# chayanchatterjee/GW-Whisper

Measured on AMD Instinct MI355X. Metric: 1s-strain segments/sec (encoder fwd), higher is better.
Workload: dtype bf16; 1 GPU; whisper-tiny encoder fwd, batch 256 log-mel (80x3000) per GPU, 1500 tokens, random-init weights (BASELINE configs[1]); global_batch=256, parallelism=dp1, encoder=tiny, streams_per_gpu=1

## Files before the change

__graft_entry__.py:

```python

from __future__ import annotations

import os
import subprocess
import sys

ROOT = os.path.dirname(os.path.abspath(__file__))
if ROOT not in sys.path:
    sys.path.insert(0, ROOT)


def build() -> None:
    csrc = os.path.join(ROOT, "gw_whisper_amd", "csrc")
    subprocess.run(["make", "-C", csrc, "-j", str(min(8, os.cpu_count() or 1))], check=True)
    asm = os.path.join(csrc, "build", "mlp_fused.s")
    subprocess.run(["/opt/rocm/bin/hipcc", "-O3", "-std=c++17", "--offload-arch=gfx950", "-ffp-contract=fast", "-mllvm",
                    "-pragma-unroll-threshold=4000000", "-S", "--cuda-device-only", os.path.join(csrc, "mlp_fused.hip"),
                    "-o", asm], check=True)
    subprocess.run([sys.executable, os.path.join(ROOT, "tools", "audit_asm_loads.py"), asm, "k_mlp_fused"], check=True)
    subprocess.run([sys.executable, os.path.join(ROOT, "tools", "audit_asm_mfma.py"), asm, "k_mlp_fused"], check=True)
    subprocess.run([sys.executable, os.path.join(ROOT, "tools", "audit_spills.py"), asm, "k_mlp_fused", "ILi1ELb1=4", "ILi3ELb1=10",
                    "ILi0ELb1=2", "ILi1ELb0=29"], check=True)
    asm4 = os.path.join(csrc, "build", "gemm_v4.s")
    subprocess.run(["/opt/rocm/bin/hipcc", "-O3", "-std=c++17", "--offload-arch=gfx950", "-ffp-contract=fast", "-S",
                    "--cuda-device-only", os.path.join(csrc, "gemm_v4.hip"), "-o", asm4], check=True)
    subprocess.run([sys.executable, os.path.join(ROOT, "tools", "audit_asm_preload.py"), asm4, "k_gemm_bf16_v4ILi2E"], check=True)
    for k in ("k_gemm_bf16_v4ILi0E", "k_gemm_bf16_v4ILi1E"):
        subprocess.run([sys.executable, os.path.join(ROOT, "tools", "audit_asm_preload.py"), asm4, k, "--no-loads"], check=True)
    for k in ("k_gemm_bf16_v4ILi3E", "k_gemm_bf16_v4ILi16E"):
        subprocess.run([sys.executable, os.path.join(ROOT, "tools", "audit_asm_preload.py"), asm4, k, "--scratch-only"], check=True)
    asmc = os.path.join(csrc, "build", "classify.s")
    subprocess.run(["/opt/rocm/bin/hipcc", "-O3", "-std=c++17", "--offload-arch=gfx950", "-ffp-contract=fast", "-S",
                    "--cuda-device-only", os.path.join(csrc, "classify.hip"), "-o", asmc], check=True)
    for k in ("k_head_fwd", "k_head_bwd_in", "k_head_bwd_w", "k_eval_accumulate"):
        subprocess.run([sys.executable, os.path.join(ROOT, "tools", "audit_asm_preload.py"), asmc, k, "--scratch-only"], check=True)
    asmd = os.path.join(csrc, "build", "detect.s")
    subprocess.run(["/opt/rocm/bin/hipcc", "-O3", "-std=c++17", "--offload-arch=gfx950", "-ffp-contract=fast", "-S",
                    "--cuda-device-only", os.path.join(csrc, "detect.hip"), "-o", asmd], check=True)
    for k in ("k_det_fwdILin1E", "k_det_fwdILi0E", "k_det_fwdILi1E", "k_det_bwd_in", "k_det_bwd_w", "k_det_eval",
              "k_sel_hist", "k_sel_pick", "k_det_counts"):
        subprocess.run([sys.executable, os.path.join(ROOT, "tools", "audit_asm_preload.py"), asmd, k, "--scratch-only"], check=True)
    asmr = os.path.join(csrc, "build", "roc.s")
    subprocess.run(["/opt/rocm/bin/hipcc", "-O3", "-std=c++17", "--offload-arch=gfx950", "-ffp-contract=off", "-S",
                    "--cuda-device-only", os.path.join(csrc, "roc.hip"), "-o", asmr], check=True)
    for k in ("k_roc_keys", "k_roc_hist", "k_roc_scan", "k_roc_scatter", "k_roc_finish", "k_roc_groups", "k_roc_curve",
              "k_roc_bootstrap", "k_roc_band", "k_bin_eval"):
        subprocess.run([sys.executable, os.path.join(ROOT, "tools", "audit_asm_preload.py"), asmr, k, "--scratch-only"], check=True)
    import gw_whisper_amd
    lib = gw_whisper_amd.lib()
    assert lib.gww_version() >= 107


def smoke() -> None:
    import numpy as np
    import torch

    from gw_whisper_amd import ops, synth
    from gw_whisper_amd.encoder import WhisperConfig, WhisperEncoder
    from oracle import encoder as oenc
    from oracle import logmel as olm

    assert torch.cuda.is_available(), "smoke() needs a GPU"
    dev = torch.device("cuda:0")
    wave = synth.strain_segments(2, seed=21)
    mel = ops.logmel(torch.from_numpy(wave).to(dev))
    mel_ref = olm.log_mel(wave)
    err_mel = float(np.abs(mel.cpu().numpy() - mel_ref).max())
    assert err_mel < 1e-4, f"log-mel mismatch {err_mel}"

    cfg = WhisperConfig(128, 2, 2, 512)
    sd = synth.encoder_state_dict(128, 2, 2, 512, seed=3)
    ref = oenc.encoder_forward(sd, mel_ref, oenc.EncCfg(128, 2, 2, 512))
    for prec, tol in (("fp32", 2e-3), ("bf16", 6e-2)):
        enc = WhisperEncoder.from_numpy_state_dict(sd, cfg, precision=prec).to(dev)
        with torch.no_grad():
            out = enc(mel).last_hidden_state
            last = enc.last_token(mel)
        torch.cuda.synchronize()
        err = float(np.abs(out.cpu().numpy() - ref).max())
        err_last = float(np.abs(last.cpu().numpy() - ref[:, -1]).max())
        print(f"smoke[{prec}]: max|hidden - oracle| = {err:.3e}, last-token {err_last:.3e}, log-mel {err_mel:.3e}")
        assert err < tol and err_last < tol, f"encoder[{prec}] mismatch {err} / {err_last}"
    d, L, H, F = synth.ENCODER_SIZES["tiny"]
    sd = synth.encoder_state_dict(d, L, H, F, seed=5)
    ref = oenc.encoder_forward(sd, mel_ref[:1], oenc.EncCfg(d, L, H, F), dtype=np.float32)
    enc = WhisperEncoder.from_numpy_state_dict(sd, WhisperConfig.named("tiny"), precision="bf16").to(dev)
    with torch.no_grad():
        out = enc(mel[:1]).last_hidden_state
    torch.cuda.synchronize()
    err = float(np.abs(out.cpu().numpy() - ref).max())
    print(f"smoke[tiny bf16]: max|hidden - oracle| = {err:.3e} (|hidden| max {np.abs(ref).max():.2f})")
    assert err < 0.15, f"whisper-tiny bf16 mismatch {err}"
    print("smoke OK")


if __name__ == "__main__":
    {"build": build, "smoke": smoke}[sys.argv[1] if len(sys.argv) > 1 else "build"]()
```

gw_whisper_amd/csrc/attention.hip:

```cpp
#include "common.h"

#include <stdlib.h>
#include <type_traits>

#ifndef GWW_ATT_EPI16
#define GWW_ATT_EPI16 1
#endif
namespace gww {

#ifdef GWW_STAMP
__device__ unsigned long long g_stamp_att[8];
#define ASTAMP_DECL unsigned long long _t0 = __builtin_amdgcn_s_memtime(); unsigned long long _acc[7] = {0, 0, 0, 0, 0, 0, 0};
#define ASTAMP(i)                                                  \
  do {                                                             \
    __builtin_amdgcn_sched_barrier(0);                             \
    const unsigned long long _t1 = __builtin_amdgcn_s_memtime();   \
    _acc[i] += _t1 - _t0;                                          \
    _t0 = _t1;                                                     \
    __builtin_amdgcn_sched_barrier(0);                             \
  } while (0)
#define ASTAMP_FLUSH                                                                 \
  if (lane == 0) {                                                                   \
    for (int _q = 0; _q < 7; ++_q) atomicAdd(&g_stamp_att[_q], _acc[_q]);            \
    atomicAdd(&g_stamp_att[7], 1ull);                                                \
// ... 355 lines not shown
    }
#pragma unroll
    for (int g = 0; g < 2; ++g)
#pragma unroll
      for (int j = 0; j < 16; ++j) st[g][j] = __builtin_amdgcn_exp2f(st[g][j]);
    if constexpr (LATE) { if (kt + 1 < n_kt) gload(kt + 1); }
    if constexpr (VSUM) {
      float ps = 0.f;
#pragma unroll
      for (int g = 0; g < 2; ++g)
#pragma unroll
        for (int j = 0; j < 16; ++j) ps += st[g][j];
      l_run += ps;
    }
#pragma unroll
    for (int g = 0; g < 2; ++g) {
#pragma unroll
      for (int s = 0; s < 2; ++s) {
        const bf16x8 pf = cvt8(st[g], 8 * s);
        if constexpr (!VSUM) lt = __builtin_amdgcn_mfma_f32_32x32x16_bf16(ones, pf, lt, 0, 0, 0);
#pragma unroll
        for (int n = 0; n < 2; ++n) {
          const unsigned char* vb = vbase[n] + BUF * TILE_BYTES + (32 * g + 16 * s) * 128;
          const bf16x4 lo4 = __builtin_amdgcn_ds_read_tr16_b64_v4bf16((lds_bf16x4_ptr)vb);
          const bf16x4 hi4 = __builtin_amdgcn_ds_read_tr16_b64_v4bf16((lds_bf16x4_ptr)(vb + 8 * 128));
          bf16x8 vf;
          vf[0] = lo4[0]; vf[1] = lo4[1]; vf[2] = lo4[2]; vf[3] = lo4[3];
          vf[4] = hi4[0]; vf[5] = hi4[1]; vf[6] = hi4[2]; vf[7] = hi4[3];
          ot[n] = __builtin_amdgcn_mfma_f32_32x32x16_bf16(vf, pf, ot[n], 0, 0, 0);
        }
      }
    }
    if (kt + 1 < n_kt) lstore(std::integral_constant<int, BUF ^ 1>{});
    __syncthreads();
  };
  using P0 = std::integral_constant<int, 0>;
  using P1 = std::integral_constant<int, 1>;
  using Yes = std::true_type;
  using No = std::false_type;

  gload(0);
  lstore(P0{});
  __syncthreads();
  const bool ragged = (T % KB) != 0;
  if (n_kt == 1) {
    if (ragged) tile(0, P0{}, Yes{}, Yes{});
    else tile(0, P0{}, Yes{}, No{});
  } else {
    tile(0, P0{}, Yes{}, No{});
    int kt = 1;
    for (; kt + 2 <= n_kt - 1; kt += 2) {
      tile(kt, P1{}, No{}, No{});
      tile(kt + 1, P0{}, No{}, No{});
    }
    if (kt == n_kt - 2) {
      tile(kt, P1{}, No{}, No{});
      if (ragged) tile(kt + 1, P0{}, No{}, Yes{});
      else tile(kt + 1, P0{}, No{}, No{});
    } else {
      if (ragged) tile(kt, P1{}, No{}, Yes{});
      else tile(kt, P1{}, No{}, No{});
    }
  }

  const float l_tot = (VAR & 2) ? l_run + __shfl_xor(l_run, 32, 64) : lt[0];
  const float inv = 1.0f / l_tot;
  if (lse && q_row < T && hh == 0)
    lse[((long)b * H + h) * T + q_row] = (m_run + __log2f(l_tot)) * 0.69314718055994530942f;
  if (q_row < T) {
    unsigned short* orow = ctx + ((long)b * T + q_row) * d + h * DH;
#pragma unroll
    for (int n = 0; n < 2; ++n)
#pragma unroll
      for (int c = 0; c < 4; ++c) {
        const int dh = 32 * n + 8 * c + 4 * hh;
        u32x2 o = {pack2bf(ot[n][4 * c] * inv, ot[n][4 * c + 1] * inv),
                   pack2bf(ot[n][4 * c + 2] * inv, ot[n][4 * c + 3] * inv)};
        *reinterpret_cast<u32x2*>(orow + dh) = o;
      }
  }
}

#endif
#ifndef GWW_ATT_NBUF
#define GWW_ATT_NBUF 2
#endif
template <int MINW, bool MSUM, bool NOMAX>
__global__ __launch_bounds__(256, MINW) void k_attention_dma_bf16(const unsigned short* __restrict__ qkv,
                                                                 unsigned short* __restrict__ ctx,
                                                                 float* __restrict__ lse, int T, int H, int q_tiles,
                                                                 int qt0) {
  constexpr int NB = GWW_ATT_NBUF;
  __shared__ __attribute__((aligned(16))) unsigned char lds[NB * 2 * KB * DH * 2];
  constexpr int TILE_BYTES = KB * DH * 2, NW = 4;
  typedef __attribute__((address_space(3))) void* lds_ptr;
  typedef const __attribute__((address_space(1))) void* g_ptr;
  const int tid = threadIdx.x, lane = tid & 63, wave = tid >> 6;
  const int wave_u = __builtin_amdgcn_readfirstlane(wave);
  const unsigned nblk = gridDim.x, per = nblk >> 3;
  const unsigned wid = blockIdx.x < 8 * per ? (blockIdx.x & 7) * per + (blockIdx.x >> 3) : blockIdx.x;
  const int qt = qt0 + wid % q_tiles;
  const int bh = wid / q_tiles;
  const int b = bh / H, h = bh - b * H;
  const int d = H * DH;
  const long row_stride = 3L * d;
  const unsigned short* base = qkv + (long)b * T * row_stride;
  const unsigned short* qp = base + h * DH;
  const unsigned short* kp = base + d + h * DH;
  const unsigned short* vp = base + 2 * d + h * DH;
  const int r = lane & 31, hh = lane >> 5;
  const int q_row = qt * (NW * 32) + wave * 32 + r;
  const int q_ld = q_row < T ? q_row : T - 1;
  const bool wave_live = qt * (NW * 32) + wave_u * 32 < T;
  bf16x8 qf[4];
#pragma unroll
  for (int s = 0; s < 4; ++s) qf[s] = *reinterpret_cast<const bf16x8*>(qp + (long)q_ld * row_stride + 16 * s + 8 * hh);

  const int n_kt = (T + KB - 1) / KB;
  const bool ragged = (T % KB) != 0;
  unsigned koff[2], voff[2];
#pragma unroll
  for (int j = 0; j < 2; ++j) {
    const int row = 8 * (2 * wave + j) + (lane >> 3), pos = lane & 7;
    koff[j] = (unsigned)(row * (int)row_stride * 2 + ((pos ^ ((row >> 1) & 7)) << 4));
    voff[j] = (unsigned)(row * (int)row_stride * 2 + ((pos ^ (((row >> 1) & 1) << 2)) << 4));
  }
  auto dma = [&](int kt, auto buf_c) {
    constexpr int BUF = decltype(buf_c)::value;
    const char* kb = reinterpret_cast<const char*>(kp + (long)kt * KB * row_stride);
    const char* vb = reinterpret_cast<const char*>(vp + (long)kt * KB * row_stride);
    unsigned char* dk = lds + BUF * TILE_BYTES + (2 * wave_u) * 1024;
    unsigned char* dv = dk + NB * TILE_BYTES;
    if constexpr (NB == 3) {
      const unsigned mk = (unsigned)(unsigned long long)(lds_ptr)dk, mv = (unsigned)(unsigned long long)(lds_ptr)dv;
      unsigned ko[2], vo[2];
      if (kt != n_kt - 1 || !ragged) {
        ko[0] = koff[0]; ko[1] = koff[1]; vo[0] = voff[0]; vo[1] = voff[1];
      } else {
        const int last_row = T - 1 - kt * KB;
#pragma unroll
        for (int j = 0; j < 2; ++j) {
          const int row = 8 * (2 * wave + j) + (lane >> 3), pos = lane & 7;
          const int rc = row < last_row ? row : last_row;
          ko[j] = (unsigned)(rc * (int)row_stride * 2 + ((pos ^ ((row >> 1) & 7)) << 4));
          vo[j] = (unsigned)(rc * (int)row_stride * 2 + ((pos ^ (((row >> 1) & 1) << 2)) << 4));
        }
      }
#pragma unroll
      for (int j = 0; j < 2; ++j) {
        asm volatile("s_mov_b32 m0, %2\n\ts_nop 0\n\tglobal_load_lds_dwordx4 %0, %1" : : "v"(ko[j]), "s"(kb), "s"(mk + 1024u * j) : "memory");
        asm volatile("s_mov_b32 m0, %2\n\ts_nop 0\n\tglobal_load_lds_dwordx4 %0, %1" : : "v"(vo[j]), "s"(vb), "s"(mv + 1024u * j) : "memory");
      }
    } else if (kt != n_kt - 1 || !ragged) {
#pragma unroll
      for (int j = 0; j < 2; ++j) {
        __builtin_amdgcn_global_load_lds((g_ptr)(kb + koff[j]), (lds_ptr)(dk + j * 1024), 16, 0, 0);
        __builtin_amdgcn_global_load_lds((g_ptr)(vb + voff[j]), (lds_ptr)(dv + j * 1024), 16, 0, 0);
      }
    } else {
      const int last_row = T - 1 - kt * KB;
#pragma unroll
      for (int j = 0; j < 2; ++j) {
        const int row = 8 * (2 * wave + j) + (lane >> 3), pos = lane & 7;
        const int rc = row < last_row ? row : last_row;
        const unsigned ko = (unsigned)(rc * (int)row_stride * 2 + ((pos ^ ((row >> 1) & 7)) << 4));
        const unsigned vo = (unsigned)(rc * (int)row_stride * 2 + ((pos ^ (((row >> 1) & 1) << 2)) << 4));
// ... 114 lines not shown
      }
    }
    if constexpr (!MSUM) l_run += ps;
#pragma unroll
    for (int g = 0; g < 2; ++g) {
      if (MASKED && g == 1 && !g1_live) continue;
#pragma unroll
      for (int s = 0; s < 2; ++s) {
        const bf16x8 pf = cvt8(st[g], 8 * s);
        if constexpr (MSUM) lt = __builtin_amdgcn_mfma_f32_32x32x16_bf16(ones, pf, lt, 0, 0, 0);
#pragma unroll
        for (int n = 0; n < 2; ++n) {
          const unsigned char* vb = vbase[n] + BUF * TILE_BYTES + (32 * g + 16 * s) * 128;
          const bf16x4 lo4 = __builtin_amdgcn_ds_read_tr16_b64_v4bf16((lds_bf16x4_ptr)vb);
          const bf16x4 hi4 = __builtin_amdgcn_ds_read_tr16_b64_v4bf16((lds_bf16x4_ptr)(vb + 8 * 128));
          bf16x8 vf;
          vf[0] = lo4[0]; vf[1] = lo4[1]; vf[2] = lo4[2]; vf[3] = lo4[3];
          vf[4] = hi4[0]; vf[5] = hi4[1]; vf[6] = hi4[2]; vf[7] = hi4[3];
          ot[n] = __builtin_amdgcn_mfma_f32_32x32x16_bf16(vf, pf, ot[n], 0, 0, 0);
        }
      }
    }
    }
    if constexpr (NB == 3) {
      if (kt + 2 < n_kt) asm volatile("s_waitcnt vmcnt(4)\n\ts_barrier" ::: "memory");
      else asm volatile("s_waitcnt vmcnt(0)\n\ts_barrier" ::: "memory");
    } else {
      __syncthreads();
    }
  };
  using P0 = std::integral_constant<int, 0>;
  using P1 = std::integral_constant<int, 1>;
  using Yes = std::true_type;
  using No = std::false_type;

  if constexpr (NB == 3) {
    using P2 = std::integral_constant<int, 2>;
    dma(0, P0{});
    if (n_kt > 1) {
      dma(1, P1{});
      asm volatile("s_waitcnt vmcnt(4)\n\ts_barrier" ::: "memory");
    } else {
      asm volatile("s_waitcnt vmcnt(0)\n\ts_barrier" ::: "memory");
    }
#pragma unroll
    for (int s4 = 0; s4 < 4; ++s4) asm volatile("" : "+v"(qf[s4]));
    tile(0, P0{}, Yes{}, No{}, n_kt == 1 && ragged);
    for (int kt = 1; kt < n_kt; kt += 3) {
      tile(kt, P1{}, No{}, No{}, ragged && kt == n_kt - 1);
      if (kt + 1 < n_kt) tile(kt + 1, P2{}, No{}, No{}, ragged && kt + 1 == n_kt - 1);
      if (kt + 2 < n_kt) tile(kt + 2, P0{}, No{}, No{}, ragged && kt + 2 == n_kt - 1);
    }
  } else {
    dma(0, P0{});
    __syncthreads();
    if (n_kt == 1) {
      if (ragged) tile(0, P0{}, Yes{}, Yes{});
      else tile(0, P0{}, Yes{}, No{});
    } else {
      tile(0, P0{}, Yes{}, No{});
      int kt = 1;
      for (; kt + 2 <= n_kt - 1; kt += 2) {
        tile(kt, P1{}, No{}, No{});
        tile(kt + 1, P0{}, No{}, No{});
      }
      if (kt == n_kt - 2) {
        tile(kt, P1{}, No{}, No{});
        if (ragged) tile(kt + 1, P0{}, No{}, Yes{});
        else tile(kt + 1, P0{}, No{}, No{});
      } else {
        if (ragged) tile(kt, P1{}, No{}, Yes{});
        else tile(kt, P1{}, No{}, No{});
      }
    }
  }

  float l_tot;
  if constexpr (MSUM) {
    l_tot = lt[0];
  } else {
    const auto sw = __builtin_amdgcn_permlane32_swap(__float_as_uint(l_run), __float_as_uint(l_run), false, false);
    l_tot = __uint_as_float(sw[0]) + __uint_as_float(sw[1]);
  }
  const float inv = 1.0f / l_tot;
  if (lse && q_row < T && hh == 0)
    lse[((long)b * H + h) * T + q_row] = (m_run + __log2f(l_tot)) * 0.69314718055994530942f;
#if GWW_ATT_EPI16
  {
    unsigned short* orow = ctx + ((long)b * T + q_row) * d + h * DH;
#pragma unroll
    for (int n = 0; n < 2; ++n)
#pragma unroll
      for (int cp = 0; cp < 2; ++cp) {
        const int c0 = 2 * cp, c1 = 2 * cp + 1;
        const unsigned a0 = pack2bf(ot[n][4 * c0] * inv, ot[n][4 * c0 + 1] * inv), a1 = pack2bf(ot[n][4 * c0 + 2] * inv, ot[n][4 * c0 + 3] * inv);
        const unsigned b0 = pack2bf(ot[n][4 * c1] * inv, ot[n][4 * c1 + 1] * inv), b1 = pack2bf(ot[n][4 * c1 + 2] * inv, ot[n][4 * c1 + 3] * inv);
        const auto s0 = __builtin_amdgcn_permlane32_swap(a0, b0, false, false);
        const auto s1 = __builtin_amdgcn_permlane32_swap(a1, b1, false, false);
        u32x4 o = {s0[0], s1[0], s0[1], s1[1]};
        if (q_row < T) *reinterpret_cast<u32x4*>(orow + 32 * n + 8 * (hh ? c1 : c0)) = o;
      }
  }
#else
  if (q_row < T) {
    unsigned short* orow = ctx + ((long)b * T + q_row) * d + h * DH;
#pragma unroll
    for (int n = 0; n < 2; ++n)
#pragma unroll
      for (int c = 0; c < 4; ++c) {
        const int dh = 32 * n + 8 * c + 4 * hh;
        u32x2 o = {pack2bf(ot[n][4 * c] * inv, ot[n][4 * c + 1] * inv),
                   pack2bf(ot[n][4 * c + 2] * inv, ot[n][4 * c + 3] * inv)};
        *reinterpret_cast<u32x2*>(orow + dh) = o;
      }
  }
#endif
}

#ifdef GWW_LAB
constexpr int PP_SLOTS = 4;
#ifndef GWW_PP_PRIO
#define GWW_PP_PRIO 0
#endif
template <int MODE>
__global__ __launch_bounds__(MODE == 1 ? 256 : 512, 1) void k_attention_pp_bf16(const unsigned short* __restrict__ qkv,
                                                              unsigned short* __restrict__ ctx,
                                                              float* __restrict__ lse, int T, int H, int q_tiles,
                                                              int qt0) {
  constexpr int TILE_BYTES = KB * DH * 2;
  __shared__ __attribute__((aligned(16))) unsigned char lds[2 * PP_SLOTS * TILE_BYTES];
  typedef __attribute__((address_space(3))) void* lds_ptr;
  typedef const __attribute__((address_space(1))) void* g_ptr;
  const int tid = threadIdx.x, lane = tid & 63;
  const int wave = __builtin_amdgcn_readfirstlane(tid >> 6);
  const bool g1 = wave >= 4;
  constexpr int NWV = MODE == 1 ? 4 : 8, PPW = 8 / NWV;
  const unsigned nblk = gridDim.x, per = nblk >> 3;
  const unsigned wid = blockIdx.x < 8 * per ? (blockIdx.x & 7) * per + (blockIdx.x >> 3) : blockIdx.x;
  const int qt = qt0 + wid % q_tiles;
  const int bh = wid / q_tiles;
  const int b = bh / H, h = bh - b * H;
  const int d = H * DH;
  const long row_stride = 3L * d;
  const unsigned short* base = qkv + (long)b * T * row_stride;
  const unsigned short* qp = base + h * DH;
  const unsigned short* kp = base + d + h * DH;
  const unsigned short* vp = base + 2 * d + h * DH;
  const int r = lane & 31, hh = lane >> 5;
  const int q_row = qt * (NWV * 32) + wave * 32 + r;
  const int q_ld = q_row < T ? q_row : T - 1;
  bf16x8 qf[4];
#pragma unroll
  for (int s = 0; s < 4; ++s) qf[s] = *reinterpret_cast<const bf16x8*>(qp + (long)q_ld * row_stride + 16 * s + 8 * hh);

  const int n_kt = (T + KB - 1) / KB;
  const bool ragged = (T % KB) != 0;
  const int dpos = lane & 7;
  int drow[PPW];
  unsigned koff[PPW], voff[PPW];
#pragma unroll
  for (int j = 0; j < PPW; ++j) {
    drow[j] = 8 * (wave + NWV * j) + (lane >> 3);
    koff[j] = (unsigned)(drow[j] * (int)row_stride * 2 + ((dpos ^ ((drow[j] >> 1) & 7)) << 4));
    voff[j] = (unsigned)(drow[j] * (int)row_stride * 2 + ((dpos ^ (((drow[j] >> 1) & 1) << 2)) << 4));
  }
  auto dma = [&](int kt) {
    const char* kb = reinterpret_cast<const char*>(kp + (long)kt * KB * row_stride);
    const char* vb = reinterpret_cast<const char*>(vp + (long)kt * KB * row_stride);
    if (kt != n_kt - 1 || !ragged) {
#pragma unroll
      for (int j = 0; j < PPW; ++j) {
        unsigned char* dk = lds + (kt & (PP_SLOTS - 1)) * TILE_BYTES + (wave + NWV * j) * 1024;
        __builtin_amdgcn_global_load_lds((g_ptr)(kb + koff[j]), (lds_ptr)dk, 16, 0, 0);
        __builtin_amdgcn_global_load_lds((g_ptr)(vb + voff[j]), (lds_ptr)(dk + PP_SLOTS * TILE_BYTES), 16, 0, 0);
      }
    } else {
      const int last_row = T - 1 - kt * KB;
#pragma unroll
      for (int j = 0; j < PPW; ++j) {
        unsigned char* dk = lds + (kt & (PP_SLOTS - 1)) * TILE_BYTES + (wave + NWV * j) * 1024;
        const int rc = drow[j] < last_row ? drow[j] : last_row;
        const unsigned ko = (unsigned)(rc * (int)row_stride * 2 + ((dpos ^ ((drow[j] >> 1) & 7)) << 4));
        const unsigned vo = (unsigned)(rc * (int)row_stride * 2 + ((dpos ^ (((drow[j] >> 1) & 1) << 2)) << 4));
        __builtin_amdgcn_global_load_lds((g_ptr)(kb + ko), (lds_ptr)dk, 16, 0, 0);
        __builtin_amdgcn_global_load_lds((g_ptr)(vb + vo), (lds_ptr)(dk + PP_SLOTS * TILE_BYTES), 16, 0, 0);
      }
    }
  };

  const int tr_q = (lane & 15) >> 2, tr_p = lane & 3;
  const int tr_colbyte = (((lane & 31) >> 4) * 16 + 4 * tr_p) * 2;
  const unsigned char* kbase[4];
#pragma unroll
  for (int s = 0; s < 4; ++s) kbase[s] = lds + k_off(r, 2 * s + hh);
  const unsigned char* vbase[2];
#pragma unroll
  for (int n = 0; n < 2; ++n) vbase[n] = lds + PP_SLOTS * TILE_BYTES + v_off(4 * hh + tr_q, 64 * n + tr_colbyte);

  f32x16 ot[2], st[2];
// ... 420 lines not shown
  using No = std::false_type;
  auto tile_rt = [&](int kt, bool masked) {
    switch (kt & 3) {
      case 0: if (masked) tile(kt, std::integral_constant<int, 0>{}, No{}, Yes{}); else tile(kt, std::integral_constant<int, 0>{}, No{}, No{}); break;
      case 1: if (masked) tile(kt, std::integral_constant<int, 1>{}, No{}, Yes{}); else tile(kt, std::integral_constant<int, 1>{}, No{}, No{}); break;
      case 2: if (masked) tile(kt, std::integral_constant<int, 2>{}, No{}, Yes{}); else tile(kt, std::integral_constant<int, 2>{}, No{}, No{}); break;
      default: if (masked) tile(kt, std::integral_constant<int, 3>{}, No{}, Yes{}); else tile(kt, std::integral_constant<int, 3>{}, No{}, No{}); break;
    }
  };

  dma(0);
  if (n_kt > 1) {
    dma(1);
    asm volatile("s_waitcnt vmcnt(2)" ::: "memory");
  } else {
    asm volatile("s_waitcnt vmcnt(0)" ::: "memory");
  }
  __builtin_amdgcn_s_barrier();
  if (g1) __builtin_amdgcn_s_barrier();
  if (GWW_PP_PRIO == 2 && g1) __builtin_amdgcn_s_setprio(1);
  if (n_kt == 1 && ragged) tile(0, std::integral_constant<int, 0>{}, Yes{}, Yes{});
  else tile(0, std::integral_constant<int, 0>{}, Yes{}, No{});
  {
    int kt = 1;
    for (; kt + 4 <= n_kt - 1; kt += 4) {
      tile(kt, std::integral_constant<int, 1>{}, No{}, No{});
      tile(kt + 1, std::integral_constant<int, 2>{}, No{}, No{});
      tile(kt + 2, std::integral_constant<int, 3>{}, No{}, No{});
      tile(kt + 3, std::integral_constant<int, 0>{}, No{}, No{});
    }
    for (; kt < n_kt; ++kt) tile_rt(kt, ragged && kt == n_kt - 1);
  }
  pv_reads((n_kt - 1) & 3);
  pv_mfma();
  if (!g1) __builtin_amdgcn_s_barrier();
  ASTAMP(6);
  ASTAMP_FLUSH
  }

  float l_tot;
  {
    const auto sw = __builtin_amdgcn_permlane32_swap(__float_as_uint(l_run), __float_as_uint(l_run), false, false);
    l_tot = __uint_as_float(sw[0]) + __uint_as_float(sw[1]);
  }
  const float inv = 1.0f / l_tot;
  if (lse && q_row < T && hh == 0)
    lse[((long)b * H + h) * T + q_row] = (m_run + __log2f(l_tot)) * 0.69314718055994530942f;
  {
    unsigned short* orow = ctx + ((long)b * T + q_row) * d + h * DH;
#pragma unroll
    for (int n = 0; n < 2; ++n)
#pragma unroll
      for (int cp = 0; cp < 2; ++cp) {
        const int c0 = 2 * cp, c1 = 2 * cp + 1;
        const unsigned a0 = pack2bf(ot[n][4 * c0] * inv, ot[n][4 * c0 + 1] * inv), a1 = pack2bf(ot[n][4 * c0 + 2] * inv, ot[n][4 * c0 + 3] * inv);
        const unsigned b0 = pack2bf(ot[n][4 * c1] * inv, ot[n][4 * c1 + 1] * inv), b1 = pack2bf(ot[n][4 * c1 + 2] * inv, ot[n][4 * c1 + 3] * inv);
        const auto s0 = __builtin_amdgcn_permlane32_swap(a0, b0, false, false);
        const auto s1 = __builtin_amdgcn_permlane32_swap(a1, b1, false, false);
        u32x4 o = {s0[0], s1[0], s0[1], s1[1]};
        if (q_row < T) *reinterpret_cast<u32x4*>(orow + 32 * n + 8 * (hh ? c1 : c0)) = o;
      }
  }
}

#endif
bool attention_log2q_enabled() {
  static const bool off = lab_int("GWW_ATT_LOG2Q", 1) == 0;
  return !off;
}

int launch_attention_bf16(const void* qkv, void* ctx, int B, int T, int H, hipStream_t s, float* lse,
                          bool last_tile_only, bool q_log2) {
  GWW_REQUIRE(qkv && ctx, "attention_bf16: NULL operand");
  GWW_REQUIRE(B >= 0 && T > 0 && H > 0, "attention_bf16: bad shape B=%d T=%d H=%d", B, T, H);
  GWW_REQUIRE((((uintptr_t)qkv) & 15) == 0 && (((uintptr_t)ctx) & 15) == 0, "attention_bf16: 16-byte alignment");
  if (B == 0) return GWW_OK;
#ifdef GWW_LAB
  if (q_log2 && !last_tile_only && lab_int("GWW_ATT_W64", 0) != 0) return launch_attention_w64_bf16(qkv, ctx, B, T, H, s, lse);
#endif
  const unsigned short* in = (const unsigned short*)qkv;
  unsigned short* out = (unsigned short*)ctx;
#ifdef GWW_LAB
  const int nw_env = (int)lab_int("GWW_ATT_WAVES", 0);
  const int var_env = (int)lab_int("GWW_ATT_VAR", 7);
  const bool pp = q_log2 && var_env >= 8;
  const int nw = ((nw_env == 8 && !q_log2) || (pp && var_env == 8)) ? 8 : 4;
#else
  const int nw = 4;
#endif
  const int all_tiles = (T + nw * 32 - 1) / (nw * 32);
  const int q_tiles = last_tile_only ? 1 : all_tiles, qt0 = last_tile_only ? all_tiles - 1 : 0;
  const long blocks = (long)q_tiles * B * H;
  GWW_REQUIRE(blocks < 2147483647L, "attention_bf16: grid too large");
#define GWW_DMA(MW, MS, NM) hipLaunchKernelGGL((k_attention_dma_bf16<MW, MS, NM>), dim3((unsigned)blocks), dim3(256), 0, s, in, out, lse, T, H, q_tiles, qt0)
#ifdef GWW_LAB
  if (pp && var_env >= 9) {
    hipLaunchKernelGGL((k_attention_pp_bf16<1>), dim3((unsigned)blocks), dim3(256), 0, s, in, out, lse, T, H, q_tiles, qt0);
  } else if (pp) {
    hipLaunchKernelGGL((k_attention_pp_bf16<0>), dim3((unsigned)blocks), dim3(512), 0, s, in, out, lse, T, H, q_tiles, qt0);
  } else if (q_log2) {
    const int var = var_env & 7;
#define GWW_L2(VV) hipLaunchKernelGGL((k_attention_l2_bf16<4, VV>), dim3((unsigned)blocks), dim3(256), 0, s, in, out, lse, T, H, q_tiles, qt0)
    switch (var) {
      case 0: GWW_L2(0); break;
      case 1: GWW_L2(1); break;
      case 2: GWW_L2(2); break;
      case 3: GWW_L2(3); break;
      case 4: GWW_DMA(3, false, false); break;
      case 5: GWW_DMA(4, false, false); break;
      case 6: GWW_DMA(3, true, false); break;
      default: GWW_DMA(3, false, true); break;
    }
#undef GWW_L2
  } else if (nw == 8) {
    hipLaunchKernelGGL(k_attention_bf16<8>, dim3((unsigned)blocks), dim3(512), 0, s, in, out, lse, T, H, q_tiles, qt0);
  } else
#else
  if (q_log2) {
    GWW_DMA(3, false, true);
  } else
#endif
  {
    hipLaunchKernelGGL(k_attention_bf16<4>, dim3((unsigned)blocks), dim3(256), 0, s, in, out, lse, T, H, q_tiles, qt0);
  }
#undef GWW_DMA
  GWW_LAUNCH_CHECK();
  return GWW_OK;
}

constexpr int FKB = 32;
constexpr int FLDS = DH + 1;

__global__ __launch_bounds__(256) void k_attention_f32(const float* __restrict__ qkv, float* __restrict__ ctx,
                                                       int T, int H, int q_tiles) {
  __shared__ float Ks[FKB][FLDS];
  __shared__ float Vs[FKB][FLDS];
  const int tid = threadIdx.x, lane = tid & 63, wave = tid >> 6;
  const int qt = blockIdx.x % q_tiles;
  const int bh = blockIdx.x / q_tiles;
  const int b = bh / H, h = bh - b * H;
  const int d = H * DH;
  const long row_stride = 3L * d;
  const float* base = qkv + (long)b * T * row_stride;
  const float* qp = base + h * DH;
  const float* kp = base + d + h * DH;
  const float* vp = base + 2 * d + h * DH;
  const int r = lane & 31, hh = lane >> 5;
  const int q_row = qt * QB + wave * 32 + r;
  const int q_ld = q_row < T ? q_row : T - 1;

  float qf[32];
#pragma unroll
  for (int s = 0; s < 32; ++s) qf[s] = qp[(long)q_ld * row_stride + 2 * s + hh];

  f32x16 ot[2];
#pragma unroll
  for (int n = 0; n < 2; ++n)
#pragma unroll
    for (int j = 0; j < 16; ++j) ot[n][j] = 0.f;
  float m_run = -INFINITY, l_run = 0.f;

  const int n_kt = (T + FKB - 1) / FKB;
  for (int kt = 0; kt < n_kt; ++kt) {
#pragma unroll
    for (int i = 0; i < 2; ++i) {
      const int c = tid + 256 * i, row = c >> 4, col = (c & 15) * 4;
      int key = kt * FKB + row;
      if (key >= T) key = T - 1;
      const float4 kv = *reinterpret_cast<const float4*>(kp + (long)key * row_stride + col);
      const float4 vv = *reinterpret_cast<const float4*>(vp + (long)key * row_stride + col);
      Ks[row][col] = kv.x; Ks[row][col + 1] = kv.y; Ks[row][col + 2] = kv.z; Ks[row][col + 3] = kv.w;
      Vs[row][col] = vv.x; Vs[row][col + 1] = vv.y; Vs[row][col + 2] = vv.z; Vs[row][col + 3] = vv.w;
    }
    __syncthreads();
    f32x16 st;
#pragma unroll
    for (int j = 0; j < 16; ++j) st[j] = 0.f;
#pragma unroll
    for (int s = 0; s < 32; ++s)
      st = __builtin_amdgcn_mfma_f32_32x32x2f32(Ks[r][2 * s + hh], qf[s], st, 0, 0, 0);
    if (kt == n_kt - 1 && (T % FKB) != 0) {
#pragma unroll
      for (int j = 0; j < 16; ++j) {
        const int key = kt * FKB + (j & 3) + 8 * (j >> 2) + 4 * hh;
        if (key >= T) st[j] = -INFINITY;
      }
    }
    float tmax = st[0];
#pragma unroll
    for (int j = 1; j < 16; ++j) tmax = fmaxf(tmax, st[j]);
    tmax = fmaxf(tmax, __shfl_xor(tmax, 32, 64));
    const float m_new = fmaxf(m_run, tmax);
    const float alpha = expf(m_run - m_new);
    float psum = 0.f;
#pragma unroll
    for (int j = 0; j < 16; ++j) {
      st[j] = expf(st[j] - m_new);
      psum += st[j];
    }
    l_run = l_run * alpha + psum;
    m_run = m_new;
#pragma unroll
    for (int n = 0; n < 2; ++n)
#pragma unroll
      for (int j = 0; j < 16; ++j) ot[n][j] *= alpha;
#pragma unroll
    for (int rho = 0; rho < 16; ++rho) {
      const int key = (rho & 3) + 8 * (rho >> 2) + 4 * hh;
// ... 181 lines not shown
```

Baseline: 25860 segments/s.

## Add half-tile attention kernel with lazy rescale and XCD-aware block remap

```diff
diff --git a/__graft_entry__.py b/__graft_entry__.py
--- a/__graft_entry__.py
+++ b/__graft_entry__.py
@@ -46,6 +46,11 @@
     for k in ("k_roc_keys", "k_roc_hist", "k_roc_scan", "k_roc_scatter", "k_roc_finish", "k_roc_groups", "k_roc_curve",
               "k_roc_bootstrap", "k_roc_band", "k_bin_eval"):
         subprocess.run([sys.executable, os.path.join(ROOT, "tools", "audit_asm_preload.py"), asmr, k, "--scratch-only"], check=True)
+    asma = os.path.join(csrc, "build", "attention.s")
+    subprocess.run(["/opt/rocm/bin/hipcc", "-O3", "-std=c++17", "--offload-arch=gfx950", "-ffp-contract=fast", "-S",
+                    "--cuda-device-only", os.path.join(csrc, "attention.hip"), "-o", asma], check=True)
+    subprocess.run([sys.executable, os.path.join(ROOT, "tools", "audit_spills.py"), asma, "k_attention_h32_bf16", "--max-vgprs=128",
+                    "--no-compiler-vmcnt-in-loops"], check=True)
     import gw_whisper_amd
     lib = gw_whisper_amd.lib()
     assert lib.gww_version() >= 107
diff --git a/gw_whisper_amd/csrc/attention.hip b/gw_whisper_amd/csrc/attention.hip
--- a/gw_whisper_amd/csrc/attention.hip
+++ b/gw_whisper_amd/csrc/attention.hip
@@ -461,6 +461,43 @@
 }
 
 #endif
+__device__ __forceinline__ void att_dma_finish(const f32x16 (&ot)[2], float l_tot, float m_run, unsigned short* __restrict__ ctx,
+                                               float* __restrict__ lse, int b, int h, int H, int T, int d, int q_row, int hh) {
+  const float inv = 1.0f / l_tot;
+  if (lse && q_row < T && hh == 0)
+    lse[((long)b * H + h) * T + q_row] = (m_run + __log2f(l_tot)) * 0.69314718055994530942f;
+#if GWW_ATT_EPI16
+  {
+    unsigned short* orow = ctx + ((long)b * T + q_row) * d + h * DH;
+#pragma unroll
+    for (int n = 0; n < 2; ++n)
+#pragma unroll
+      for (int cp = 0; cp < 2; ++cp) {
+        const int c0 = 2 * cp, c1 = 2 * cp + 1;
+        const unsigned a0 = pack2bf(ot[n][4 * c0] * inv, ot[n][4 * c0 + 1] * inv), a1 = pack2bf(ot[n][4 * c0 + 2] * inv, ot[n][4 * c0 + 3] * inv);
+        const unsigned b0 = pack2bf(ot[n][4 * c1] * inv, ot[n][4 * c1 + 1] * inv), b1 = pack2bf(ot[n][4 * c1 + 2] * inv, ot[n][4 * c1 + 3] * inv);
+        const auto s0 = __builtin_amdgcn_permlane32_swap(a0, b0, false, false);
+        const auto s1 = __builtin_amdgcn_permlane32_swap(a1, b1, false, false);
+        u32x4 o = {s0[0], s1[0], s0[1], s1[1]};
+        if (q_row < T) *reinterpret_cast<u32x4*>(orow + 32 * n + 8 * (hh ? c1 : c0)) = o;
+      }
+  }
+#else
+  if (q_row < T) {
+    unsigned short* orow = ctx + ((long)b * T + q_row) * d + h * DH;
+#pragma unroll
+    for (int n = 0; n < 2; ++n)
+#pragma unroll
+      for (int c = 0; c < 4; ++c) {
+        const int dh = 32 * n + 8 * c + 4 * hh;
+        u32x2 o = {pack2bf(ot[n][4 * c] * inv, ot[n][4 * c + 1] * inv),
+                   pack2bf(ot[n][4 * c + 2] * inv, ot[n][4 * c + 3] * inv)};
+        *reinterpret_cast<u32x2*>(orow + dh) = o;
+      }
+  }
+#endif
+}
+
 #ifndef GWW_ATT_NBUF
 #define GWW_ATT_NBUF 2
 #endif
@@ -741,39 +778,178 @@
     const auto sw = __builtin_amdgcn_permlane32_swap(__float_as_uint(l_run), __float_as_uint(l_run), false, false);
     l_tot = __uint_as_float(sw[0]) + __uint_as_float(sw[1]);
   }
-  const float inv = 1.0f / l_tot;
-  if (lse && q_row < T && hh == 0)
-    lse[((long)b * H + h) * T + q_row] = (m_run + __log2f(l_tot)) * 0.69314718055994530942f;
-#if GWW_ATT_EPI16
-  {
-    unsigned short* orow = ctx + ((long)b * T + q_row) * d + h * DH;
-#pragma unroll
-    for (int n = 0; n < 2; ++n)
-#pragma unroll
-      for (int cp = 0; cp < 2; ++cp) {
-        const int c0 = 2 * cp, c1 = 2 * cp + 1;
-        const unsigned a0 = pack2bf(ot[n][4 * c0] * inv, ot[n][4 * c0 + 1] * inv), a1 = pack2bf(ot[n][4 * c0 + 2] * inv, ot[n][4 * c0 + 3] * inv);
-        const unsigned b0 = pack2bf(ot[n][4 * c1] * inv, ot[n][4 * c1 + 1] * inv), b1 = pack2bf(ot[n][4 * c1 + 2] * inv, ot[n][4 * c1 + 3] * inv);
-        const auto s0 = __builtin_amdgcn_permlane32_swap(a0, b0, false, false);
-        const auto s1 = __builtin_amdgcn_permlane32_swap(a1, b1, false, false);
-        u32x4 o = {s0[0], s1[0], s0[1], s1[1]};
-        if (q_row < T) *reinterpret_cast<u32x4*>(orow + 32 * n + 8 * (hh ? c1 : c0)) = o;
-      }
-  }
-#else
-  if (q_row < T) {
-    unsigned short* orow = ctx + ((long)b * T + q_row) * d + h * DH;
-#pragma unroll
-    for (int n = 0; n < 2; ++n)
-#pragma unroll
-      for (int c = 0; c < 4; ++c) {
-        const int dh = 32 * n + 8 * c + 4 * hh;
-        u32x2 o = {pack2bf(ot[n][4 * c] * inv, ot[n][4 * c + 1] * inv),
-                   pack2bf(ot[n][4 * c + 2] * inv, ot[n][4 * c + 3] * inv)};
-        *reinterpret_cast<u32x2*>(orow + dh) = o;
-      }
-  }
-#endif
+  att_dma_finish(ot, l_tot, m_run, ctx, lse, b, h, H, T, d, q_row, hh);
+}
+
+__global__ __launch_bounds__(256, 4) void k_attention_h32_bf16(const unsigned short* __restrict__ qkv,
+                                                              unsigned short* __restrict__ ctx,
+                                                              float* __restrict__ lse, int T, int H, int q_tiles,
+                                                              int qt0) {
+  __shared__ __attribute__((aligned(16))) unsigned char lds[2 * 2 * KB * DH * 2];
+  constexpr int TILE_BYTES = KB * DH * 2, NW = 4;
+  typedef __attribute__((address_space(3))) void* lds_ptr;
+  typedef const __attribute__((address_space(3))) bf16x8* lds_bf16x8_ptr;
+  typedef bf16x4 __attribute__((address_space(3))) * lds_bf16x4_ptr;
+  const int tid = threadIdx.x, lane = tid & 63, wave = tid >> 6;
+  const int wave_u = __builtin_amdgcn_readfirstlane(wave);
+  const unsigned nblk = gridDim.x, per = nblk >> 3;
+  const unsigned wid = blockIdx.x < 8 * per ? (blockIdx.x & 7) * per + (blockIdx.x >> 3) : blockIdx.x;
+  const int qt = qt0 + wid % q_tiles;
+  const int bh = wid / q_tiles;
+  const int b = bh / H, h = bh - b * H;
+  const int d = H * DH;
+  const long row_stride = 3L * d;
+  const unsigned short* base = qkv + (long)b * T * row_stride;
+  const unsigned short* qp = base + h * DH;
+  const unsigned short* kp = base + d + h * DH;
+  const unsigned short* vp = base + 2 * d + h * DH;
+  const int r = lane & 31, hh = lane >> 5;
+  const int q_row = qt * (NW * 32) + wave * 32 + r;
+  const int q_ld = q_row < T ? q_row : T - 1;
+  const bool wave_live = qt * (NW * 32) + wave_u * 32 < T;
+  bf16x8 qf[4];
+#pragma unroll
+  for (int s = 0; s < 4; ++s) qf[s] = *reinterpret_cast<const bf16x8*>(qp + (long)q_ld * row_stride + 16 * s + 8 * hh);
+
+  const int n_kt = (T + KB - 1) / KB;
+  const bool ragged = (T % KB) != 0;
+  const unsigned lds0 = (unsigned)(unsigned long long)(lds_ptr)lds;
+  auto dma = [&](int kt, auto buf_c) {
+    constexpr int BUF = decltype(buf_c)::value;
+    const char* kb = reinterpret_cast<const char*>(kp + (long)kt * KB * row_stride);
+    const char* vb = reinterpret_cast<const char*>(vp + (long)kt * KB * row_stride);
+    const unsigned mk = lds0 + BUF * TILE_BYTES + (2 * wave_u) * 1024, mv = mk + 2 * TILE_BYTES;
+    const int last_row = (kt == n_kt - 1 && ragged) ? T - 1 - kt * KB : KB - 1;
+#pragma unroll
+    for (int j = 0; j < 2; ++j) {
+      const int row = 8 * (2 * wave + j) + (lane >> 3), pos = lane & 7;
+      const int rc = row < last_row ? row : last_row;
+      const unsigned ko = (unsigned)(rc * (int)row_stride * 2 + ((pos ^ ((row >> 1) & 7)) << 4));
+      const unsigned vo = (unsigned)(rc * (int)row_stride * 2 + ((pos ^ (((row >> 1) & 1) << 2)) << 4));
+      asm volatile("s_mov_b32 m0, %2\n\ts_nop 0\n\tglobal_load_lds_dwordx4 %0, %1" : : "v"(ko), "s"(kb), "s"(mk + 1024u * j) : "memory");
+      asm volatile("s_mov_b32 m0, %2\n\ts_nop 0\n\tglobal_load_lds_dwordx4 %0, %1" : : "v"(vo), "s"(vb), "s"(mv + 1024u * j) : "memory");
+    }
+  };
+
+  const int tr_q = (lane & 15) >> 2, tr_p = lane & 3;
+  const int tr_colbyte = (((lane & 31) >> 4) * 16 + 4 * tr_p) * 2;
+  const unsigned kof0 = k_off(r, hh), vof0 = v_off(4 * hh + tr_q, tr_colbyte);
+
+  f32x16 ot[2];
+#pragma unroll
+  for (int j = 0; j < 16; ++j) { ot[0][j] = 0.f; ot[1][j] = 0.f; }
+  unsigned mref_pk = 0;
+  float l_run = 0.f, m_run = 0.f;
+
+  auto half = [&](int kt, auto buf_c, auto g_c, auto first_c, bool masked) {
+    constexpr int BUF = decltype(buf_c)::value, G = decltype(g_c)::value;
+    constexpr bool FIRST = decltype(first_c)::value;
+    f32x16 st;
+    auto score = [&]() {
+#pragma unroll
+      for (int j = 0; j < 16; ++j) st[j] = 0.f;
+      if constexpr (!FIRST) {
+        const u32x4 o4 = {0x3f803f80u, 0x3f803f80u, 0x3f803f80u, 0x3f803f80u}, m4 = {mref_pk, 0u, 0u, 0u};
+        st = __builtin_amdgcn_mfma_f32_32x32x16_bf16(__builtin_bit_cast(bf16x8, o4), __builtin_bit_cast(bf16x8, m4), st, 0, 0, 0);
+      }
+#pragma unroll
+      for (int s = 0; s < 4; ++s) {
+        const bf16x8 kf = *(lds_bf16x8_ptr)(lds0 + (kof0 ^ (unsigned)(s << 5)) + (unsigned)(BUF * TILE_BYTES + G * (32 * 128)));
+        st = __builtin_amdgcn_mfma_f32_32x32x16_bf16(kf, qf[s], st, 0, 0, 0);
+      }
+      if (masked) {
+#pragma unroll
+        for (int j = 0; j < 16; ++j) {
+          const int key = kt * KB + 32 * G + (j & 3) + 8 * (j >> 2) + 4 * hh;
+          if (key >= T) st[j] = -INFINITY;
+        }
+      }
+    };
+    auto rebase = [&]() {
+      float tmax = st[0];
+#pragma unroll
+      for (int j = 1; j < 16; ++j) tmax = fmaxf(tmax, st[j]);
+      {
+        const auto sw = __builtin_amdgcn_permlane32_swap(__float_as_uint(tmax), __float_as_uint(tmax), false, false);
+        tmax = fmaxf(__uint_as_float(sw[0]), __uint_as_float(sw[1]));
+      }
+      const float want = m_run + (FIRST ? tmax : fmaxf(tmax, 0.f));
+      const __bf16 hi = (__bf16)(-want);
+      const __bf16 lo = (__bf16)(-want - (float)hi);
+      const float m_new = -((float)hi + (float)lo);
+      const float dm = m_new - m_run;
+      m_run = m_new;
+      mref_pk = hh == 0 ? ((unsigned)__builtin_bit_cast(unsigned short, hi) | ((unsigned)__builtin_bit_cast(unsigned short, lo) << 16)) : 0u;
+      if constexpr (!FIRST) {
+        const float alpha = __builtin_amdgcn_exp2f(-dm);
+        l_run *= alpha;
+#pragma unroll
+        for (int j = 0; j < 16; ++j) { ot[0][j] *= alpha; ot[1][j] *= alpha; }
+      }
+#pragma unroll
+      for (int j = 0; j < 16; ++j) st[j] -= dm;
+    };
+    float ps;
+    auto exps = [&]() {
+      ps = 0.f;
+#pragma unroll
+      for (int j = 0; j < 16; ++j) {
+        st[j] = __builtin_amdgcn_exp2f(st[j]);
+        ps += st[j];
+      }
+    };
+    score();
+    if constexpr (FIRST) rebase();
+    exps();
+    if constexpr (!FIRST) {
+      if (__builtin_expect(__builtin_amdgcn_ballot_w64(!(ps <= 2981.0f)) != 0, 0)) {
+        score();
+        rebase();
+        exps();
+      }
+    }
+    l_run += ps;
+#pragma unroll
+    for (int s = 0; s < 2; ++s) {
+      const bf16x8 pf = cvt8(st, 8 * s);
+#pragma unroll
+      for (int n = 0; n < 2; ++n) {
+        const unsigned va = lds0 + (vof0 ^ (unsigned)(n << 6)) + (unsigned)((2 + BUF) * TILE_BYTES + (32 * G + 16 * s) * 128);
+        const bf16x4 lo4 = __builtin_amdgcn_ds_read_tr16_b64_v4bf16((lds_bf16x4_ptr)va);
+        const bf16x4 hi4 = __builtin_amdgcn_ds_read_tr16_b64_v4bf16((lds_bf16x4_ptr)(va + 8 * 128));
+        bf16x8 vf;
+        vf[0] = lo4[0]; vf[1] = lo4[1]; vf[2] = lo4[2]; vf[3] = lo4[3];
+        vf[4] = hi4[0]; vf[5] = hi4[1]; vf[6] = hi4[2]; vf[7] = hi4[3];
+        ot[n] = __builtin_amdgcn_mfma_f32_32x32x16_bf16(vf, pf, ot[n], 0, 0, 0);
+      }
+    }
+  };
+  using P0 = std::integral_constant<int, 0>;
+  using P1 = std::integral_constant<int, 1>;
+  using Yes = std::true_type;
+  using No = std::false_type;
+  auto tile = [&](int kt, auto buf_c, auto first_c, bool masked) {
+    constexpr int BUF = decltype(buf_c)::value;
+    if (kt + 1 < n_kt) dma(kt + 1, std::integral_constant<int, BUF ^ 1>{});
+    if (wave_live) {
+      half(kt, buf_c, P0{}, first_c, masked);
+      if (!masked || (T - kt * KB) > 32) half(kt, buf_c, P1{}, No{}, masked);
+    }
+    asm volatile("s_waitcnt vmcnt(0)\n\ts_barrier" ::: "memory");
+  };
+
+  dma(0, P0{});
+  asm volatile("s_waitcnt vmcnt(0)\n\ts_barrier" ::: "memory");
+#pragma unroll
+  for (int s4 = 0; s4 < 4; ++s4) asm volatile("" : "+v"(qf[s4]));
+  tile(0, P0{}, Yes{}, n_kt == 1 && ragged);
+  for (int kt = 1; kt < n_kt; kt += 2) {
+    tile(kt, P1{}, No{}, ragged && kt == n_kt - 1);
+    if (kt + 1 < n_kt) tile(kt + 1, P0{}, No{}, ragged && kt + 1 == n_kt - 1);
+  }
+
+  const auto sw = __builtin_amdgcn_permlane32_swap(__float_as_uint(l_run), __float_as_uint(l_run), false, false);
+  att_dma_finish(ot, __uint_as_float(sw[0]) + __uint_as_float(sw[1]), m_run, ctx, lse, b, h, H, T, d, q_row, hh);
 }
 
 #ifdef GWW_LAB
@@ -1360,8 +1536,8 @@
   unsigned short* out = (unsigned short*)ctx;
 #ifdef GWW_LAB
   const int nw_env = (int)lab_int("GWW_ATT_WAVES", 0);
-  const int var_env = (int)lab_int("GWW_ATT_VAR", 7);
-  const bool pp = q_log2 && var_env >= 8;
+  const int var_env = (int)lab_int("GWW_ATT_VAR", 10);
+  const bool pp = q_log2 && (var_env == 8 || var_env == 9);
   const int nw = ((nw_env == 8 && !q_log2) || (pp && var_env == 8)) ? 8 : 4;
 #else
   const int nw = 4;
@@ -1371,8 +1547,11 @@
   const long blocks = (long)q_tiles * B * H;
   GWW_REQUIRE(blocks < 2147483647L, "attention_bf16: grid too large");
 #define GWW_DMA(MW, MS, NM) hipLaunchKernelGGL((k_attention_dma_bf16<MW, MS, NM>), dim3((unsigned)blocks), dim3(256), 0, s, in, out, lse, T, H, q_tiles, qt0)
+#define GWW_H32() hipLaunchKernelGGL(k_attention_h32_bf16, dim3((unsigned)blocks), dim3(256), 0, s, in, out, lse, T, H, q_tiles, qt0)
 #ifdef GWW_LAB
-  if (pp && var_env >= 9) {
+  if (q_log2 && var_env >= 10) {
+    GWW_H32();
+  } else if (pp && var_env >= 9) {
     hipLaunchKernelGGL((k_attention_pp_bf16<1>), dim3((unsigned)blocks), dim3(256), 0, s, in, out, lse, T, H, q_tiles, qt0);
   } else if (pp) {
     hipLaunchKernelGGL((k_attention_pp_bf16<0>), dim3((unsigned)blocks), dim3(512), 0, s, in, out, lse, T, H, q_tiles, qt0);
@@ -1395,13 +1574,14 @@
   } else
 #else
   if (q_log2) {
-    GWW_DMA(3, false, true);
+    GWW_H32();
   } else
 #endif
   {
     hipLaunchKernelGGL(k_attention_bf16<4>, dim3((unsigned)blocks), dim3(256), 0, s, in, out, lse, T, H, q_tiles, qt0);
   }
 #undef GWW_DMA
+#undef GWW_H32
   GWW_LAUNCH_CHECK();
   return GWW_OK;
 }
```

After: 25970 segments/s (median of 6 runs). No clear change (+0.5%).
